# kostas1515/object_detectors

Measured on AMD Instinct MI355X. Metric: images/sec (fwd+bwd) YOLOv3 640px bs=32, higher is better.
Workload: dtype bf16; 1 GPU; YOLOv3 Darknet-53 training step (fwd+loss+bwd+SGD step), synthetic COCO 640px, per-GPU bs=32, 7 GT/img, random-init weights; global_batch=32, parallelism=dp1

## Files before the change

include/mi355det.h:

```cpp
#ifndef MI355DET_H
#define MI355DET_H

#include <stddef.h>
#include <stdint.h>

#ifdef __cplusplus
extern "C" {
#endif

#define MI355DET_OK 0
#define MI355DET_EINVAL (-1)
#define MI355DET_ELAUNCH (-2)
#define MI355DET_EWORKSPACE (-3)

#define MI355DET_MAX_SCALES 4
#define MI355DET_MAX_ANCHORS 8

const char* mi355det_last_error(void);
int mi355det_debug_set(int key, int value);
int mi355det_debug_ptr(int key, void* ptr);
int mi355det_version(void);

typedef struct {
  int32_t num_scales, na, num_classes, pad0;
// ... 156 lines not shown
                           void* workspace, size_t workspace_bytes, void* stream);

typedef struct {
  int32_t n, h, w, cin;
  int32_t ho, wo, cout;
  int32_t ksize, stride, pad;
  int32_t in_ld, out_ld;
} mi355det_conv_shape;

int mi355det_conv_fwd(const mi355det_conv_shape* s, const void* x, const void* w, const float* bias,
                      void* y, int out_f32, float* stats, int32_t cout_pad, void* stream);
typedef struct {
  const float* scale;
  const float* shift;
  const void* residual;
  int32_t residual_ld;
  int32_t relu;
  int64_t out_image_stride;
  float slope;
} mi355det_conv_epilogue;
int mi355det_conv_fwd_ex(const mi355det_conv_shape* s, const void* x, const void* w, const mi355det_conv_epilogue* e,
                         void* y, int out_f32, int32_t cout_pad, void* stream);
int mi355det_conv_autotune_mode(int on);

typedef struct {
  uint32_t table;
  int32_t value;
  uint64_t key;
} mi355det_tune_entry;
size_t mi355det_tune_export(void* buf, size_t cap);
int mi355det_tune_import(const void* buf, size_t bytes, int replace);
int mi355det_tune_lock(int on);
int mi355det_tune_clear(void);
int mi355det_conv_stats_rows(const mi355det_conv_shape* s, int32_t cout_pad);
int mi355det_stem_im2col(const float* img, void* out, int32_t n, int32_t h, int32_t w, void* stream);

int mi355det_stem_l1_rows(int32_t n, int32_t h, int32_t w);
int mi355det_stem_l1_fwd(const float* img, const void* w0, const float* scale_shift0, float slope, const void* w1, void* a0,
                         int32_t a0_ld, void* z1, int32_t z1_ld, float* stats, int32_t n, int32_t h, int32_t w, void* stream);
int mi355det_stem_l1_fwd_eval(const float* img, const void* w0, const float* scale_shift0, float slope, const void* w1,
                              const float* scale_shift1, void* a1, int32_t a1_ld, int32_t n, int32_t h, int32_t w, void* stream);
int mi355det_stem_rows(int32_t n, int32_t h, int32_t w);
int mi355det_stem_fwd_stats(const float* img, const void* w, float* partial, int32_t n, int32_t h, int32_t wd, void* stream);
int mi355det_stem_fwd_apply(const float* img, const void* w, const float* scale_shift, float slope, void* a, int32_t a_ld,
                            int32_t n, int32_t h, int32_t wd, void* stream);
int mi355det_stem_bwd_reduce(const float* img, const void* w, const float* scale_shift, float slope, const void* da,
// ... 385 lines not shown
```

include/mi355det_f16.h:

```cpp
#ifndef MI355DET_F16_H
#define MI355DET_F16_H
#include "mi355det.h"
#ifdef __cplusplus
extern "C" {
#endif

int mi355det_conv_autotune_mode_f16(int on);
int mi355det_conv_dgrad_f16(const mi355det_conv_shape* s, const void* dy, const void* wt, void* dx, const void* residual, int32_t residual_ld, void* stream);
int mi355det_conv_dgrad_bn_f16(const mi355det_conv_shape* s, const void* dy, const void* wt, void* dx, const void* residual, int32_t residual_ld, const void* z, int32_t z_ld, const float* scale_shift, float slope, float* partials, void* stream);
int mi355det_conv_dgrad_bn_rows_f16(const mi355det_conv_shape* s);
int mi355det_conv_dgrad_mask_f16(const mi355det_conv_shape* s, const void* dy, const void* wt, void* dx, const void* act, int32_t act_ld, const float* scale, int32_t relu, void* stream);
size_t mi355det_conv_dgrad_workspace_f16(const mi355det_conv_shape* s);
int mi355det_conv_dgrad_ws_f16(const mi355det_conv_shape* s, const void* dy, const void* wt, void* dx, const void* residual, int32_t residual_ld, void* workspace, size_t workspace_bytes, void* stream);
int mi355det_conv_fwd_f16(const mi355det_conv_shape* s, const void* x, const void* w, const float* bias, void* y, int out_f32, float* stats, int32_t cout_pad, void* stream);
int mi355det_conv_fwd_ex_f16(const mi355det_conv_shape* s, const void* x, const void* w, const mi355det_conv_epilogue* e, void* y, int out_f32, int32_t cout_pad, void* stream);
int mi355det_conv_stats_rows_f16(const mi355det_conv_shape* s, int32_t cout_pad);
int mi355det_debug_ptr_f16(int key, void* ptr);
int mi355det_debug_set_f16(int key, int value);
size_t mi355det_dgrad_pack_elems_f16(const mi355det_conv_shape* s);
int mi355det_pack_table_build_f16(const mi355det_pack_item* items, int32_t n, void* host_table, size_t host_bytes);
size_t mi355det_pack_table_bytes_f16(const mi355det_pack_item* items, int32_t n, int32_t* n_entries, int32_t* n_blocks);
int mi355det_pack_weights_f16(const mi355det_conv_shape* s, const float* w, int w_is_ohwi, void* w_fwd, int32_t cout_pad, void* w_dgrad, void* stream);
int mi355det_pack_weights_batched_f16(const void* dev_table, int32_t n_entries, int32_t n_blocks, void* stream);
int mi355det_stem_im2col_f16(const float* img, void* out, int32_t n, int32_t h, int32_t w, void* stream);
int mi355det_unpack_wgrad_f16(const mi355det_conv_shape* s, const float* dw, float* grad, void* stream);
int mi355det_conv_wgrad_f16(const mi355det_conv_shape* s, const void* x, const void* dy, float* dw, float* dbias, void* workspace, size_t workspace_bytes, void* stream);
int mi355det_conv_wgrad_autotune_f16(const mi355det_conv_shape* s, const void* x, const void* dy, float* dw, void* workspace, size_t workspace_bytes, void* stream);
size_t mi355det_conv_wgrad_workspace_f16(const mi355det_conv_shape* s);
int mi355det_add_bf16_f16(const void* a, int32_t a_ld, const void* b, int32_t b_ld, int32_t c, int64_t pixels, void* out, int32_t out_ld, void* stream);
int mi355det_bn_act_bwd_apply_f16(const void* g1, int32_t g1_ld, const void* g2, int32_t g2_ld, const void* z, int32_t z_ld, const float* scale_shift, const float* sums, const float* gamma, int32_t c, int64_t pixels, float slope, void* dz, int32_t dz_ld, float* dgamma, float* dbeta, void* stream);
// ... 24 lines not shown
```

object_detectors_amd/_lib.py:

```python
import ctypes as C
import os

HERE = os.path.dirname(os.path.abspath(__file__))
LIB_PATH = os.environ.get("MI355DET_LIB", os.path.join(HERE, "libmi355det.so"))

MAX_SCALES, MAX_ANCHORS = 4, 8

vp, i32, i64, f32, sz = C.c_void_p, C.c_int32, C.c_int64, C.c_float, C.c_size_t


class YoloGeom(C.Structure):
    _fields_ = [("num_scales", i32), ("na", i32), ("num_classes", i32), ("pad0", i32),
                ("img_size", f32), ("ignore_thr", f32), ("iou_type", i32), ("pad1", i32),
                ("grid", i32 * MAX_SCALES), ("off", i32 * (MAX_SCALES + 1)),
                ("anchor_w", (f32 * MAX_ANCHORS) * MAX_SCALES), ("anchor_h", (f32 * MAX_ANCHORS) * MAX_SCALES)]


class HeadView(C.Structure):
    _fields_ = [("ptr", vp), ("sb", i64), ("sc", i64), ("sp", i64)]


class YoloLossCfg(C.Structure):
    _fields_ = [("lambda_iou", f32), ("lambda_xy", f32), ("lambda_wh", f32), ("lambda_conf", f32),
                ("lambda_no_conf", f32), ("lambda_cls", f32), ("alpha", f32), ("gamma", f32),
# ... 99 lines not shown
    "mi355det_roi_align": (C.c_int, [vp, vp, vp, vp, i32, vp, i32, i32, i32, i32, i32, C.c_int, i32, i32, vp, vp, vp, vp]),
    "mi355det_topk": (C.c_int, [vp, i32, i64, i64, i32, f32, vp, vp, vp, vp]),
    "mi355det_conv_fwd": (C.c_int, [P(ConvShape), vp, vp, vp, vp, C.c_int, vp, i32, vp]),
    "mi355det_conv_dgrad": (C.c_int, [P(ConvShape), vp, vp, vp, vp, i32, vp]),
    "mi355det_conv_dgrad_mask": (C.c_int, [P(ConvShape), vp, vp, vp, vp, i32, vp, i32, vp]),
    "mi355det_conv_dgrad_workspace": (sz, [P(ConvShape)]),
    "mi355det_conv_dgrad_ws": (C.c_int, [P(ConvShape), vp, vp, vp, vp, i32, vp, sz, vp]),
    "mi355det_conv_wgrad_workspace": (sz, [P(ConvShape)]),
    "mi355det_conv_wgrad_autotune": (C.c_int, [P(ConvShape), vp, vp, vp, vp, sz, vp]),
    "mi355det_conv_wgrad": (C.c_int, [P(ConvShape), vp, vp, vp, vp, vp, sz, vp]),
    "mi355det_dgrad_pack_elems": (sz, [P(ConvShape)]),
    "mi355det_pack_weights": (C.c_int, [P(ConvShape), vp, C.c_int, vp, i32, vp, vp]),
    "mi355det_pack_table_bytes": (sz, [P(PackItem), i32, P(i32), P(i32)]),
    "mi355det_pack_table_build": (C.c_int, [P(PackItem), i32, vp, sz]),
    "mi355det_pack_weights_batched": (C.c_int, [vp, i32, i32, vp]),
    "mi355det_unpack_wgrad": (C.c_int, [P(ConvShape), vp, vp, vp]),
    "mi355det_gconv_pack_elems": (sz, [P(ConvShape), i32]),
    "mi355det_gconv_pack_weights": (C.c_int, [P(ConvShape), i32, vp, C.c_int, vp, vp, vp]),
    "mi355det_gconv_fwd_ex": (C.c_int, [P(ConvShape), i32, vp, vp, P(ConvEpilogue), vp, C.c_int, vp]),
    "mi355det_gconv_dgrad": (C.c_int, [P(ConvShape), i32, vp, vp, vp, vp]),
    "mi355det_gconv_wgrad_workspace": (sz, [P(ConvShape), i32]),
    "mi355det_gconv_wgrad": (C.c_int, [P(ConvShape), i32, vp, vp, vp, vp, sz, vp]),
    "mi355det_conv_autotune_mode": (C.c_int, [C.c_int]),
    "mi355det_tune_export": (sz, [vp, sz]),
    "mi355det_tune_import": (C.c_int, [vp, sz, C.c_int]),
    "mi355det_tune_lock": (C.c_int, [C.c_int]),
    "mi355det_tune_clear": (C.c_int, []),
    "mi355det_conv_stats_rows": (C.c_int, [P(ConvShape), i32]),
    "mi355det_stem_im2col": (C.c_int, [vp, vp, i32, i32, i32, vp]),
    "mi355det_stem_rows": (C.c_int, [i32, i32, i32]),
    "mi355det_stem_l1_rows": (C.c_int, [i32, i32, i32]),
    "mi355det_stem_l1_fwd": (C.c_int, [vp, vp, vp, f32, vp, vp, i32, vp, i32, vp, i32, i32, i32, vp]),
    "mi355det_stem_l1_fwd_eval": (C.c_int, [vp, vp, vp, f32, vp, vp, vp, i32, i32, i32, i32, vp]),
    "mi355det_stem_fwd_stats": (C.c_int, [vp, vp, vp, i32, i32, i32, vp]),
    "mi355det_stem_fwd_apply": (C.c_int, [vp, vp, vp, f32, vp, i32, i32, i32, i32, vp]),
    "mi355det_stem_bwd_reduce": (C.c_int, [vp, vp, vp, f32, vp, i32, vp, i32, i32, i32, vp]),
    "mi355det_stem_bwd_apply_wgrad": (C.c_int, [vp, vp, vp, vp, f32, vp, i32, vp, vp, vp, vp, i32, i32, i32, vp]),
    "mi355det_stem_bwd_fused": (C.c_int, [vp, vp, vp, f32, vp, i32, vp, vp, vp, i32, i32, i32, vp]),
    "mi355det_stem_bwd_finish": (C.c_int, [vp, vp, vp, vp, i64, vp, vp, vp, vp]),
    "mi355det_bn_finalize": (C.c_int, [vp, i32, i32, i32, i64, vp, vp, f32, f32, vp, vp, vp, vp]),
    "mi355det_bn_eval_scale_shift": (C.c_int, [i32, vp, vp, vp, vp, f32, vp, vp]),
    "mi355det_bn_fold_partials_f64": (C.c_int, [vp, i32, i32, i32, vp, vp]),
    "mi355det_bn_finalize_f64": (C.c_int, [vp, i32, i32, i64, vp, vp, f32, f32, vp, vp, vp, vp]),
    "mi355det_conv_dgrad_bn_rows": (C.c_int, [P(ConvShape)]),
    "mi355det_conv_dgrad_bn": (C.c_int, [P(ConvShape), vp, vp, vp, vp, i32, vp, i32, vp, C.c_float, vp, vp]),
    "mi355det_bn_bwd_sum_partials": (C.c_int, [vp, i32, i32, i32, vp, vp]),
# ... 174 lines not shown
```

object_detectors_amd/csrc/conv_kernels.hip:

```cpp
#include "common.h"

#include <cstdlib>

#include <unordered_map>

#include "tune_record.h"
#include "tune_timing.h"

using namespace mi355;

#include "igemm_common.h"

extern int g_wgrad_general;
extern int g_wgrad_force_dbg;
extern int g_wgrad8_off;
extern int g_wgrad_ablate;
extern int g_dgrad_s2_off;
extern int g_conv_strict;
int mi355det_internal_dgrad_s2(const mi355det_conv_shape* s, const void* dy, const void* wt, void* dx, const void* residual, int32_t residual_ld,
                               void* stream, int probe = 0);

namespace {

#define STAMP(v) do { if (PROF) { __builtin_amdgcn_sched_barrier(0); asm volatile("s_memtime %0\n\ts_waitcnt lgkmcnt(0)" : "=s"(v) :: "memory"); __builtin_amdgcn_sched_barrier(0); } } while (0)
// ... 80 lines not shown
      }
    }
    a_voff[i] = voff;
    a_valid[i] = vm;
  }
  if (PROF) asm volatile("s_nop 0" ::"v"(a_voff[0]), "v"(a_valid[A_PER - 1]));
  STAMP(t_p2);
  int b_voff[B_PER], b_instr[B_PER];
#pragma unroll
  for (int i = 0; i < B_PER; ++i) {
    const int instr = (wid * B_PER + i) % B_INSTR;
    const int row = instr * R + lrow;
    b_instr[i] = instr;
    b_voff[i] = (row * Ktot + (cpos ^ swz<BK>(row)) * 8) * 2;
  }
  __builtin_amdgcn_s_waitcnt(0xC07F);
  STAMP(t_p3);
  __builtin_amdgcn_s_barrier();
  STAMP(t_p4);

  const int cin_steps = __builtin_amdgcn_readfirstlane((p.ksplit > 1 ? p.Cin / p.ksplit : p.Cin) / BK);
  const int c0b = sp * cin_steps * (BK * 2);
  const int ksteps = ABL == 5 ? 0 : p.T * cin_steps;
  int pf_t = 0, pf_c = 0;

  auto stage = [&](int s, int buf) {
    const int coff = c0b + pf_c * (BK * 2);
    const int soff = __builtin_amdgcn_readfirstlane(s_toff[pf_t]) + coff;
    const int boff = pf_t * (p.Cin * 2) + coff;
    char* sa = smem + buf * STAGE;
    char* sb = sa + BM * ROWB;
#pragma unroll
    for (int i = 0; i < A_PER; ++i) {
      const int instr = wid * A_PER + i;
      bufld16(rsrc_x, sa + instr * 1024, ((a_valid[i] >> pf_t) & 1u) ? a_voff[i] : OOB_VOFF, soff);
    }
#pragma unroll
    for (int i = 0; i < B_PER; ++i) bufld16(rsrc_w, sb + b_instr[i] * 1024, b_voff[i], boff);
    if (++pf_c == cin_steps) {
      pf_c = 0;
      ++pf_t;
    }
  };

  auto issue_piece = [&](int q, int boff, int soff, int tap, int buf) {
    char* sa = smem + buf * STAGE;
    char* sb = sa + BM * ROWB;
    if (q < A_PER) {
      const int instr = wid * A_PER + q;
      bufld16(rsrc_x, sa + instr * 1024, ((a_valid[q] >> tap) & 1u) ? a_voff[q] : OOB_VOFF, soff);
    } else {
      bufld16(rsrc_w, sb + b_instr[q - A_PER] * 1024, b_voff[q - A_PER], boff);
    }
  };

  f32x4_t acc[TN][TM];
#pragma unroll
  for (int i = 0; i < TN; ++i)
#pragma unroll
    for (int j = 0; j < TM; ++j) acc[i][j] = {0.f, 0.f, 0.f, 0.f};

#pragma unroll
  for (int s = 0; s < D; ++s)
    if (s < ksteps && ABL != 1) stage(s, s);

  const int fr = lane & 15, fq = lane >> 4;
  int buf = 0;
  STAMP(t_loop);
  for (int s = 0; s < ksteps; ++s) {
    STAMP(t_a);
    const int younger = min(D - 1, ksteps - 1 - s);
    if (D >= 1 && younger >= D - 1) wait_vmcnt<(D - 1 > 0 ? D - 1 : 0) * PER>();
    else if (D >= 3 && younger == D - 2) wait_vmcnt<(D - 2 > 0 ? D - 2 : 0) * PER>();
    else if (D >= 4 && younger == D - 3) wait_vmcnt<(D - 3 > 0 ? D - 3 : 0) * PER>();
    else if (D >= 5 && younger == D - 4) wait_vmcnt<(D - 4 > 0 ? D - 4 : 0) * PER>();
    else if (D >= 6 && younger == D - 5) wait_vmcnt<(D - 5 > 0 ? D - 5 : 0) * PER>();
    else wait_vmcnt<0>();
    STAMP(t_b);
    __builtin_amdgcn_s_barrier();
    STAMP(t_c);
    const bool pf = s + D < ksteps;
    const int pbuf = buf == 0 ? NST - 1 : buf - 1;
    int il_soff = 0, il_tap = 0, il_boff = 0;
    if (!ILV) {
      if (pf && ABL != 1) stage(s + D, pbuf);
    } else if (pf) {
      il_tap = pf_t;
      il_soff = __builtin_amdgcn_readfirstlane(s_toff[pf_t]) + c0b + pf_c * (BK * 2);
      il_boff = pf_t * (p.Cin * 2) + c0b + pf_c * (BK * 2);
      if (++pf_c == cin_steps) {
        pf_c = 0;
        ++pf_t;
      }
    }
    STAMP(t_d);
    const char* sa = smem + buf * STAGE;
    const char* sb = sa + BM * ROWB;
#pragma unroll
    for (int ks = 0; ks < BK / 32; ++ks) {
      st16x8_t wf[TN], af[TM];
#pragma unroll
      for (int i = 0; i < TN; ++i) {
        const int row = wn * (TN * 16) + i * 16 + fr;
        if (ABL == 2) { wf[i] = __builtin_bit_cast(st16x8_t, make_uint4(row, s, ks, i)); asm volatile("" : "+v"(wf[i])); }
        else wf[i] = *(const st16x8_t*)(sb + row * ROWB + (((ks * 4 + fq) ^ swz<BK>(row)) << 4));
      }
#pragma unroll
      for (int j = 0; j < TM; ++j) {
        const int row = wm * (TM * 16) + j * 16 + fr;
        if (ABL == 2) { af[j] = __builtin_bit_cast(st16x8_t, make_uint4(row, s, ks, j)); asm volatile("" : "+v"(af[j])); }
        else af[j] = *(const st16x8_t*)(sa + row * ROWB + (((ks * 4 + fq) ^ swz<BK>(row)) << 4));
      }
      constexpr int NMF = TN * TM * (BK / 32);
      constexpr int G = NMF / PER > 0 ? NMF / PER : 1;
#pragma unroll
      for (int i = 0; i < TN; ++i)
// ... 303 lines not shown
      const int n = (int)fdiv((unsigned)t1, p.dMH), yy = t1 - n * p.MH;
      const int iy0 = yy * p.sin, ix0 = xx * p.sin;
      voff = ((((n - n_first) * p.Hin + iy0) * p.Win + ix0) * p.ldin + (cpos ^ swz<BK>(row)) * 8) * 2;
#pragma unroll
      for (int t = 0; t < MAX_TAPS; ++t) {
        const int dyt = (int)((p.dy_pack >> (4 * t)) & 0xF) - 2, dxt = (int)((p.dx_pack >> (4 * t)) & 0xF) - 2;
        const bool ok = t < p.T && (unsigned)(iy0 + dyt) < (unsigned)p.Hin && (unsigned)(ix0 + dxt) < (unsigned)p.Win;
        vm |= ok ? (1u << t) : 0u;
      }
    }
    a_voff[i] = voff;
    a_valid[i] = vm;
  }
#pragma unroll
  for (int i = 0; i < B_PER; ++i) {
    const int instr = (wid * B_PER + i) % B_INSTR;
    const int row = instr * R + lrow;
    b_instr[i] = instr;
    b_voff[i] = (row * Ktot + (cpos ^ swz<BK>(row)) * 8) * 2;
  }
  __builtin_amdgcn_s_waitcnt(0xC07F);
  __builtin_amdgcn_s_barrier();
  const int ksteps = Ktot / BK, cin_steps = p.Cin / BK;
  int pf_t = 0, pf_c = 0;

  f32x4_t acc[TN][TM];
#pragma unroll
  for (int i = 0; i < TN; ++i)
#pragma unroll
    for (int j = 0; j < TM; ++j) acc[i][j] = {0.f, 0.f, 0.f, 0.f};

  auto piece = [&](int q, int s, int soff, int tap, int buf, bool live) {
    char* sa = smem + buf * STAGE;
    char* sb = sa + BM * ROWB;
    if (q < A_PER) {
      const bool ok = live && ((a_valid[q] >> tap) & 1u);
      bufld16(rsrc_x, sa + (wid * A_PER + q) * 1024, ok ? a_voff[q] : OOB_VOFF, soff);
    } else {
      bufld16(rsrc_w, sb + b_instr[q - A_PER] * 1024, live ? b_voff[q - A_PER] : OOB_VOFF, s * (BK * 2));
    }
  };
  {
    const int soff = __builtin_amdgcn_readfirstlane(s_toff[0]);
#pragma unroll
    for (int q = 0; q < PER; ++q) piece(q, 0, soff, 0, 0, true);
    if (++pf_c == cin_steps) {
      pf_c = 0;
      ++pf_t;
    }
  }
  const int fr = lane & 15, fq = lane >> 4;
  for (int s = 0; s < ksteps; ++s) {
    const int buf = s & 1;
    wait_vmcnt<0>();
    __builtin_amdgcn_s_barrier();
    const bool live = s + 1 < ksteps;
    const int tap = live ? pf_t : 0;
    const int soff = __builtin_amdgcn_readfirstlane(s_toff[tap]) + pf_c * (BK * 2);
    if (++pf_c == cin_steps) {
      pf_c = 0;
      ++pf_t;
    }
    const char* sa = smem + buf * STAGE;
    const char* sb = sa + BM * ROWB;
    st16x8_t wf[KS][TN], af[KS][TM];
#pragma unroll
    for (int ks = 0; ks < KS; ++ks) {
#pragma unroll
      for (int i = 0; i < TN; ++i) {
        const int row = wn * (TN * 16) + i * 16 + fr;
        wf[ks][i] = *(const st16x8_t*)(sb + row * ROWB + (((ks * 4 + fq) ^ swz<BK>(row)) << 4));
      }
#pragma unroll
      for (int j = 0; j < TM; ++j) {
        const int row = wm * (TM * 16) + j * 16 + fr;
        af[ks][j] = *(const st16x8_t*)(sa + row * ROWB + (((ks * 4 + fq) ^ swz<BK>(row)) << 4));
      }
    }
#pragma unroll
    for (int ks = 0; ks < KS; ++ks)
#pragma unroll
      for (int i = 0; i < TN; ++i)
#pragma unroll
        for (int j = 0; j < TM; ++j) {
          acc[i][j] = MI355_MFMA_16x16x32(wf[ks][i], af[ks][j], acc[i][j]);
          const int cnt = (ks * TN + i) * TM + j + 1;
          if (cnt % G == 0 && cnt / G - 1 < PER) piece(cnt / G - 1, s + 1, soff, tap, buf ^ 1, live);
        }
    if (SCHED == 1) {
      __builtin_amdgcn_sched_group_barrier(0x100, KS * (TN + TM), 0);
#pragma unroll
      for (int q = 0; q < PER; ++q) {
        __builtin_amdgcn_sched_group_barrier(0x8, G, 0);
        __builtin_amdgcn_sched_group_barrier(0x20, 1, 0);
      }
    }
  }
  __builtin_amdgcn_s_waitcnt(0xC07F);
  wait_vmcnt<0>();
  __builtin_amdgcn_s_barrier();
  igemm_epilogue<WM, WN, TM, TN, EPI>(p, acc, smem, tid, NT, true, wm, wn, lane, mt, n0, m0);
}

__global__ void pack_fwd_kernel(const float* __restrict__ w, bf16_t* __restrict__ out, int cout, int cout_pad, int cin, int cin_pad, int kk,
                                long long s_co, long long s_ci, long long s_t) {
  const long long total = (long long)cout_pad * kk * cin_pad;
  for (long long i = blockIdx.x * (long long)blockDim.x + threadIdx.x; i < total; i += (long long)gridDim.x * blockDim.x) {
    const int c = (int)(i % cin_pad);
    const int t = (int)((i / cin_pad) % kk);
    const int co = (int)(i / ((long long)cin_pad * kk));
// ... 91 lines not shown
    const int co = (int)(j % cout), tap = (int)((j / cout) % T), r = (int)(j / ((long long)cout * T));
    const int px = r / cin, ci = r - px * cin;
    const int oy = py ? tap >> 1 : 0, ox = py ? tap & 1 : tap;
    const int kh = s2cat_k(py, oy), kw = s2cat_k(px, ox);
    float v = 0.f;
    if (kh >= 0 && kw >= 0) v = w[co * s_co + ci * s_ci + (kh * 3 + kw) * s_t];
    out[i] = f2s(v);
  }
}

bf16_t* g_zero_page = nullptr;

int ensure_zero_page() {
  if (g_zero_page) return 0;
  void* p = nullptr;
  if (hipMalloc(&p, 4096) != hipSuccess) return fail(MI355DET_ELAUNCH, "%s: hipMalloc(zero page) failed", "conv");
  if (hipMemset(p, 0, 4096) != hipSuccess) return fail(MI355DET_ELAUNCH, "%s: hipMemset(zero page) failed", "conv");
  g_zero_page = (bf16_t*)p;
  return 0;
}

unsigned long long* g_dbg = nullptr;

template <int WM, int WN, int TM, int TN, int BK, int NST, int EPI, bool PROF = false, bool ILV = false, int OCC = 0, int ABL = 0>
int launch_cfg(const IgemmParams& p_in, hipStream_t st) {
  IgemmParams p = p_in;
  p.dbg = PROF ? g_dbg : nullptr;
  constexpr int BM = WM * TM * 16, BN = WN * TN * 16;
  constexpr int lds_ring = NST * (BM + BN) * BK * 2 + 64;
  constexpr int lds_epi = EPI_LDS_OFF + WM * WN * (64 * (TN * 32 + 16) + 256);
  constexpr int lds = lds_ring > lds_epi ? lds_ring : lds_epi;
  const int gm = (p.M + BM - 1) / BM, gn = p.CoutPad / BN;
  auto k = igemm_kernel<WM, WN, TM, TN, BK, NST, EPI, PROF, ILV, OCC, ABL>;
  static DeviceOnce attr_done;
  attr_done.once([&] {
    (void)hipFuncSetAttribute((const void*)k, hipFuncAttributeMaxDynamicSharedMemorySize, lds);
  });
  hipLaunchKernelGGL(k, dim3(gm * gn * (p.ksplit > 1 ? p.ksplit : 1)), dim3(WM * WN * 64), lds, st, p);
  return check_launch("igemm");
}

template <int WM, int WN, int TM, int TN, int BK, int EPI, int SCHED>
int launch_il(const IgemmParams& p, hipStream_t st) {
  constexpr int BM = WM * TM * 16, BN = WN * TN * 16;
  constexpr int lds_ring = 2 * (BM + BN) * BK * 2 + 64;
  constexpr int lds_epi = EPI_LDS_OFF + WM * WN * (64 * (TN * 32 + 16) + 256);
  constexpr int lds = lds_ring > lds_epi ? lds_ring : lds_epi;
  const int gm = (p.M + BM - 1) / BM, gn = p.CoutPad / BN;
  auto k = igemm_il_kernel<WM, WN, TM, TN, BK, EPI, SCHED>;
  static DeviceOnce attr_done;
  attr_done.once([&] {
    (void)hipFuncSetAttribute((const void*)k, hipFuncAttributeMaxDynamicSharedMemorySize, lds);
  });
  hipLaunchKernelGGL(k, dim3(gm * gn), dim3(WM * WN * 64), lds, st, p);
  return check_launch("igemm_il");
}

int g_tune = 0;

int strict_reject(int cfg, const char* why) {
  char msg[160];
  snprintf(msg, sizeof(msg), "conv: forced tile configuration %d not taken: %s (strict mode, debug key 9)", cfg, why);
  return fail(MI355DET_EINVAL, "%s", msg);
}
bool strict_forced() { return g_conv_strict && g_tune != 0; }
TuneMap& g_igemm_tuned = tune_table(TUNE_IGEMM);
// ... 38 lines not shown
  auto k = igemm_dx_kernel<WM, WN, TM, TN, EPI, NSTB, PROF, BK>;
  static DeviceOnce attr_done;
  attr_done.once([&] {
    (void)hipFuncSetAttribute((const void*)k, hipFuncAttributeMaxDynamicSharedMemorySize, lds);
  });
  hipLaunchKernelGGL(k, dim3(gm * gn), dim3(WM * WN * 64), lds, st, p);
  return check_launch("igemm_dx");
}

enum CfgReq { REQ_WIDE, REQ_DX, REQ_IG8, REQ_NARROW, REQ_NARROW_DX };
typedef int (*LaunchFn)(const IgemmParams&, hipStream_t);
struct CfgRow {
  int id;
  unsigned epis;
  int req, a, b;
  bool tuned, solo;
  LaunchFn launch;
  bool narrow() const { return req == REQ_NARROW || req == REQ_NARROW_DX; }
};
constexpr unsigned eSTATS = 1u << EPI_STATS, eF32 = 1u << EPI_F32, eRES = 1u << EPI_RES, ePLAIN = 1u << EPI_PLAIN, eAFF = 1u << EPI_AFF,
                   eBNRED = 1u << EPI_BNRED, eALL = eSTATS | eF32 | eRES | ePLAIN | eAFF | eBNRED;

template <int EPI, int ROWS>
int launch_ig8(const IgemmParams& p, hipStream_t st) { return igemm8_launch(EPI, p, st, ROWS); }

template <int EPI>
int launch_narrow(const IgemmParams& p, hipStream_t st) {
  const bool k64 = p.Cin % 64 == 0;
  if (p.CoutPad % 64 == 0) return k64 ? launch_cfg<4, 1, 4, 4, 64, 2, EPI>(p, st) : launch_cfg<4, 1, 4, 4, 32, 3, EPI>(p, st);
  if (p.CoutPad % 32 == 0) return k64 ? launch_cfg<4, 1, 4, 2, 64, 2, EPI>(p, st) : launch_cfg<4, 1, 4, 2, 32, 4, EPI>(p, st);
  return fail(MI355DET_EINVAL, "%s: padded Cout must be a multiple of 32 (got %lld)", "conv", p.CoutPad);
}

#define CFG_ROW(id, epis, req, a, b, tuned, solo, ...) \
  {id, epis, req, a, b, tuned, solo, [] { if constexpr ((((epis) >> EPI) & 1u) != 0) return (LaunchFn)(__VA_ARGS__); else return (LaunchFn) nullptr; }()}

template <int EPI>
const CfgRow* cfg_rows() {
  static const CfgRow rows[] = {
    CFG_ROW( 0, eALL,                              REQ_NARROW,      0,   0, 1, 0, launch_narrow<EPI>),
    CFG_ROW( 1, eALL,                              REQ_WIDE,      128,   0, 1, 0, launch_cfg<2, 2, 4, 4, 64, 2, EPI>),
    CFG_ROW( 2, eALL,                              REQ_WIDE,      128,   0, 1, 0, launch_cfg<2, 2, 8, 4, 32, 2, EPI>),
    CFG_ROW( 3, eALL,                              REQ_WIDE,      256,   0, 1, 1, launch_cfg<2, 4, 8, 4, 64, 2, EPI>),
    CFG_ROW( 4, eALL,                              REQ_WIDE,      128,   0, 1, 0, launch_cfg<2, 2, 4, 4, 32, 3, EPI>),
    CFG_ROW( 5, eALL,                              REQ_WIDE,      128,   0, 1, 0, launch_cfg<2, 2, 4, 4, 32, 2, EPI, false, false, 4>),
    CFG_ROW( 6, eALL,                              REQ_WIDE,      256,   0, 1, 1, launch_il<2, 4, 8, 4, 64, EPI, 0>),
    CFG_ROW(15, eALL,                              REQ_DX,        128,  64, 1, 0, launch_dx<2, 2, 4, 4, EPI>),
// ... 177 lines not shown

}

extern "C" {

int mi355det_debug_set(int key, int value) {
  if (key == 0) g_tune = value;
  if (key == 1) g_wgrad_general = value;
  if (key == 2) g_dgrad_s2_off = value;
  if (key == 3) igemm8_set_dbg_mode(value);
  if (key == 8) g_wgrad8_off = value;
  if (key == 7) g_wgrad_force_dbg = value;
  if (key == 6) g_wgrad_ablate = value;
  if (key == 5) g_s2cat_force = value;
  if (key == 9) g_conv_strict = value;
  return 0;
}

int mi355det_conv_autotune_mode(int on) {
  g_autotune_mode = on != 0;
  return 0;
}

int mi355det_debug_ptr(int key, void* ptr) {
  if (key == 0) g_dbg = (unsigned long long*)ptr;
  if (key == 1) igemm8_set_dbg((unsigned long long*)ptr);
  return 0;
}

int mi355det_conv_stats_rows(const mi355det_conv_shape* s, int32_t cout_pad) {
  (void)cout_pad;
  return s ? (int)(((long long)s->n * s->ho * s->wo + 127) / 128) : 0;
}

static int conv_fwd_impl(const mi355det_conv_shape* s, const void* x, const void* w, const float* bias, void* y, int out_f32, float* stats,
                         int32_t cout_pad, const mi355det_conv_epilogue* ex, void* stream) {
  if (int e = check_shape(s, "conv_fwd")) return e;
  if (int e = ensure_zero_page()) return e;
  if (cout_pad < s->cout) return fail(MI355DET_EINVAL, "%s: cout_pad < cout", "conv_fwd");
  if (!out_f32 && (s->cout % 8)) return fail(MI355DET_EINVAL, "%s: 16-bit outputs need cout %% 8 == 0 (got %lld)", "conv_fwd", s->cout);
  IgemmParams p{};
  p.x = (const bf16_t*)x;
  p.w = (const bf16_t*)w;
  p.y = y;
  p.bias = bias;
  p.stats = stats;
// ... 521 lines not shown
```

object_detectors_amd/csrc/f16_names.h:

```cpp
#pragma once
#define mi355det_conv_autotune_mode mi355det_conv_autotune_mode_f16
#define mi355det_conv_dgrad mi355det_conv_dgrad_f16
#define mi355det_conv_dgrad_bn mi355det_conv_dgrad_bn_f16
#define mi355det_conv_dgrad_bn_rows mi355det_conv_dgrad_bn_rows_f16
#define mi355det_conv_dgrad_mask mi355det_conv_dgrad_mask_f16
#define mi355det_conv_dgrad_workspace mi355det_conv_dgrad_workspace_f16
#define mi355det_conv_dgrad_ws mi355det_conv_dgrad_ws_f16
#define mi355det_conv_fwd mi355det_conv_fwd_f16
#define mi355det_conv_fwd_ex mi355det_conv_fwd_ex_f16
#define mi355det_conv_stats_rows mi355det_conv_stats_rows_f16
#define mi355det_debug_ptr mi355det_debug_ptr_f16
#define mi355det_debug_set mi355det_debug_set_f16
#define mi355det_dgrad_pack_elems mi355det_dgrad_pack_elems_f16
#define mi355det_pack_table_build mi355det_pack_table_build_f16
#define mi355det_pack_table_bytes mi355det_pack_table_bytes_f16
#define mi355det_pack_weights mi355det_pack_weights_f16
#define mi355det_pack_weights_batched mi355det_pack_weights_batched_f16
#define mi355det_stem_im2col mi355det_stem_im2col_f16
#define mi355det_unpack_wgrad mi355det_unpack_wgrad_f16
#define mi355det_conv_wgrad mi355det_conv_wgrad_f16
#define mi355det_conv_wgrad_autotune mi355det_conv_wgrad_autotune_f16
#define mi355det_conv_wgrad_workspace mi355det_conv_wgrad_workspace_f16
#define mi355det_add_bf16 mi355det_add_bf16_f16
#define mi355det_bn_act_bwd_apply mi355det_bn_act_bwd_apply_f16
// ... 32 lines not shown
```

object_detectors_amd/csrc/igemm8_kernels.hip:

```cpp
#include "igemm_common.h"

struct SkParams {
  unsigned long long* dbg;
};

namespace {

typedef __attribute__((ext_vector_type(4))) unsigned u32x4_t;

constexpr int kBM = 256, kBN = 256, kBK = 64, kROWB = 128;
constexpr int kHALF = 128 * kROWB;
constexpr int kSTAGE = 4 * kHALF;
constexpr int kLDS = 2 * kSTAGE;

template <int N>
__device__ __forceinline__ void wait_vm() {
  asm volatile("s_waitcnt vmcnt(%0)" ::"n"(N) : "memory");
}
template <int PROF_>
__device__ __forceinline__ void bar_b() {
  if (PROF_ == 8) return;
  asm volatile("" ::: "memory");
  __builtin_amdgcn_s_barrier();
  asm volatile("" ::: "memory");
// ... 102 lines not shown
            for (int t = 0; t < MAX_TAPS; ++t) {
              if (t >= p.T) break;
              const int dyt = (int)((p.dy_pack >> (4 * t)) & 0xF) - 2, dxt = (int)((p.dx_pack >> (4 * t)) & 0xF) - 2;
              const bool ok = (unsigned)(iy0 + dyt) < (unsigned)p.Hin && (unsigned)(ix0 + dxt) < (unsigned)p.Win;
              vm |= ok ? (1u << t) : 0u;
            }
          }
          a_voff[h][i] = voff;
          a_valid[h][i] = vm;
        }
        {
          const int row = (r2 >> 5) * 64 + h * 32 + (r2 & 31);
          b_voff[h][i] = (row * Ktot + (cpos ^ sw) * 8) * 2;
        }
      }

    int xrd = (wm * 64 + fr) * kROWB + ((fq ^ fsw) << 4);
    int wrd = 2 * kHALF + (wn * 32 + fr) * kROWB + ((fq ^ fsw) << 4);

    auto tap_off = [&](int tap) {
      const int dyt = (int)((p.dy_pack >> (4 * tap)) & 0xF) - 2, dxt = (int)((p.dx_pack >> (4 * tap)) & 0xF) - 2;
      return ((dyt * p.Win + dxt) * p.ldin + p.tap_pad) * 2;
    };
    int pf_s = k0, pf_t = k0 / cin_steps, pf_c = k0 - pf_t * cin_steps;
    struct Slot { int tap, soffx, soffw, live; };
    auto next_slot = [&]() {
      Slot s;
      s.live = pf_s < k1;
      s.tap = s.live ? pf_t : 31;
      s.soffx = s.live ? tap_off(pf_t) + pf_c * (kBK * 2) : 0;
      s.soffw = s.live ? pf_s * (kBK * 2) : 0;
      ++pf_s;
      if (++pf_c == cin_steps) {
        pf_c = 0;
        ++pf_t;
      }
      return s;
    };
    auto issue_x = [&](const Slot& s, int h, int buf) {
      if (PROF == 3) return;
      char* dst = smem + buf * kSTAGE + h * kHALF + (2 * wid) * 1024;
#pragma unroll
      for (int i = 0; i < 2; ++i) bufld16(rsrc_x, dst + i * 1024, ((a_valid[h][i] >> s.tap) & 1u) ? a_voff[h][i] : OOB_VOFF, s.soffx);
    };
    auto issue_w = [&](const Slot& s, int h, int buf) {
      if (PROF == 3) return;
      char* dst = smem + buf * kSTAGE + (2 + h) * kHALF + (2 * wid) * 1024;
#pragma unroll
      for (int i = 0; i < 2; ++i) bufld16(rsrc_w, dst + i * 1024, s.live ? b_voff[h][i] : OOB_VOFF, s.soffw);
    };

    f32x4_t acc[TN][TM];
#pragma unroll
    for (int i = 0; i < TN; ++i)
#pragma unroll
      for (int j = 0; j < TM; ++j) acc[i][j] = {0.f, 0.f, 0.f, 0.f};

    Slot s1 = next_slot();
    issue_x(s1, 0, 0);
// ... 333 lines not shown
```

object_detectors_amd/csrc/igemm_common.h:

```cpp
#pragma once
#include "common.h"

using namespace mi355;

typedef __attribute__((ext_vector_type(4))) float f32x4_t;
typedef __attribute__((ext_vector_type(8))) unsigned short u16x8_t;

#define MAX_TAPS 9

struct FastDiv {
  unsigned mul, shift;
};
static FastDiv make_fastdiv(unsigned d) {
  FastDiv f;
  unsigned l = 0;
  while ((1ull << l) < d) ++l;
  f.shift = l;
  f.mul = (unsigned)(((1ull << 32) * ((1ull << l) - d)) / d + 1);
  return f;
}
__device__ __forceinline__ unsigned fdiv(unsigned n, const FastDiv f) { return (__umulhi(f.mul, n) + n) >> f.shift; }

struct IgemmParams {
  const bf16_t* x;
// ... 3 lines not shown
  const float* scale;
  int relu;
  long long ynstride;
  const bf16_t* z;
  const float* ss;
  int ldz;
  float slope;
  float* stats;
  const bf16_t* res;
  const bf16_t* zero;
  int M, MH, MW;
  int Hin, Win, ldin, Cin, sin;
  int Hout, Wout, ldout, so, oy0, ox0;
  int sox;
  int Cout, CoutPad, ldres;
  int T;
  int dy[MAX_TAPS], dx[MAX_TAPS];
  FastDiv dMW, dMH;
  int tap_pad;
  unsigned long long dy_pack, dx_pack;
  int ksplit;
  long long ysplit;
  int lin_in, lin_out;
  unsigned long long* dbg;
};

enum { EPI_STATS = 0, EPI_F32 = 1, EPI_RES = 2, EPI_PLAIN = 3, EPI_AFF = 4, EPI_BNRED = 5 };
#define EPI_LDS_OFF 4096
#define EPI_LDS_BYTES(nwaves) (EPI_LDS_OFF + (nwaves) * (64 * (8 * 16 * 2 + 16) + 256))

bool igemm8_applicable(const IgemmParams& p);
int igemm8_launch(int epi, const IgemmParams& p, hipStream_t st, int rows = 256);
void igemm8_set_dbg(unsigned long long* ptr);
void igemm8_set_dbg_mode(int mode);

namespace {

__device__ __forceinline__ void glds16(const void* gsrc, void* lds_dst_uniform) {
  __builtin_amdgcn_global_load_lds((const __attribute__((address_space(1))) void*)gsrc,
                                   (__attribute__((address_space(3))) void*)lds_dst_uniform, 16, 0, 0);
}

typedef __attribute__((ext_vector_type(4))) int srd_t;
__device__ __forceinline__ srd_t make_srd(const void* base, unsigned num_records) {
  const unsigned long long a = (unsigned long long)base;
  srd_t r;
// ... 329 lines not shown
```

Baseline: 1163 images/s.

## Add chunk-major K-loop ordering for implicit-GEMM convolutions

Introduces a KWalk abstraction so the K reduction in the implicit-GEMM conv kernels can iterate channel-chunk-major (all taps of a channel chunk, then the next chunk) instead of tap-major. This becomes the default whenever a conv has multiple taps and multiple channel chunks, except for stride-2 inputs with BK=32. The intent is better cache locality for activation loads, since consecutive K-steps then read neighbouring spatial positions of the same channel slice. The change adds extra index arithmetic per step, and the weight offset is now derived from tap and chunk rather than the linear step counter. The wgrad/dgrad kernels that take this path also depend on the packed weight layout matching the tap*Cin+chunk indexing.

```diff
diff --git a/include/mi355det.h b/include/mi355det.h
--- a/include/mi355det.h
+++ b/include/mi355det.h
@@ -202,6 +202,7 @@
 int mi355det_conv_fwd_ex(const mi355det_conv_shape* s, const void* x, const void* w, const mi355det_conv_epilogue* e,
                          void* y, int out_f32, int32_t cout_pad, void* stream);
 int mi355det_conv_autotune_mode(int on);
+int mi355det_conv_korder(int order);
 
 typedef struct {
   uint32_t table;
diff --git a/include/mi355det_f16.h b/include/mi355det_f16.h
--- a/include/mi355det_f16.h
+++ b/include/mi355det_f16.h
@@ -6,6 +6,7 @@
 #endif
 
 int mi355det_conv_autotune_mode_f16(int on);
+int mi355det_conv_korder_f16(int order);
 int mi355det_conv_dgrad_f16(const mi355det_conv_shape* s, const void* dy, const void* wt, void* dx, const void* residual, int32_t residual_ld, void* stream);
 int mi355det_conv_dgrad_bn_f16(const mi355det_conv_shape* s, const void* dy, const void* wt, void* dx, const void* residual, int32_t residual_ld, const void* z, int32_t z_ld, const float* scale_shift, float slope, float* partials, void* stream);
 int mi355det_conv_dgrad_bn_rows_f16(const mi355det_conv_shape* s);
diff --git a/object_detectors_amd/_lib.py b/object_detectors_amd/_lib.py
--- a/object_detectors_amd/_lib.py
+++ b/object_detectors_amd/_lib.py
@@ -145,6 +145,7 @@
     "mi355det_gconv_wgrad_workspace": (sz, [P(ConvShape), i32]),
     "mi355det_gconv_wgrad": (C.c_int, [P(ConvShape), i32, vp, vp, vp, vp, sz, vp]),
     "mi355det_conv_autotune_mode": (C.c_int, [C.c_int]),
+    "mi355det_conv_korder": (C.c_int, [C.c_int]),
     "mi355det_tune_export": (sz, [vp, sz]),
     "mi355det_tune_import": (C.c_int, [vp, sz, C.c_int]),
     "mi355det_tune_lock": (C.c_int, [C.c_int]),
diff --git a/object_detectors_amd/csrc/conv_kernels.hip b/object_detectors_amd/csrc/conv_kernels.hip
--- a/object_detectors_amd/csrc/conv_kernels.hip
+++ b/object_detectors_amd/csrc/conv_kernels.hip
@@ -126,25 +126,22 @@
   const int cin_steps = __builtin_amdgcn_readfirstlane((p.ksplit > 1 ? p.Cin / p.ksplit : p.Cin) / BK);
   const int c0b = sp * cin_steps * (BK * 2);
   const int ksteps = ABL == 5 ? 0 : p.T * cin_steps;
-  int pf_t = 0, pf_c = 0;
+  KWalk kw{0, 0};
 
   auto stage = [&](int s, int buf) {
-    const int coff = c0b + pf_c * (BK * 2);
-    const int soff = __builtin_amdgcn_readfirstlane(s_toff[pf_t]) + coff;
-    const int boff = pf_t * (p.Cin * 2) + coff;
+    const int tap = kw.tap;
+    const int soff = kslot_xoff(kw, __builtin_amdgcn_readfirstlane(s_toff[tap]), c0b, BK);
+    const int boff = kslot_woff(kw, p.Cin, c0b, BK);
     char* sa = smem + buf * STAGE;
     char* sb = sa + BM * ROWB;
 #pragma unroll
     for (int i = 0; i < A_PER; ++i) {
       const int instr = wid * A_PER + i;
-      bufld16(rsrc_x, sa + instr * 1024, ((a_valid[i] >> pf_t) & 1u) ? a_voff[i] : OOB_VOFF, soff);
+      bufld16(rsrc_x, sa + instr * 1024, ((a_valid[i] >> tap) & 1u) ? a_voff[i] : OOB_VOFF, soff);
     }
 #pragma unroll
     for (int i = 0; i < B_PER; ++i) bufld16(rsrc_w, sb + b_instr[i] * 1024, b_voff[i], boff);
-    if (++pf_c == cin_steps) {
-      pf_c = 0;
-      ++pf_t;
-    }
+    kwalk_next(kw, p.T, cin_steps, p.korder);
   };
 
   auto issue_piece = [&](int q, int boff, int soff, int tap, int buf) {
@@ -189,13 +186,10 @@
     if (!ILV) {
       if (pf && ABL != 1) stage(s + D, pbuf);
     } else if (pf) {
-      il_tap = pf_t;
-      il_soff = __builtin_amdgcn_readfirstlane(s_toff[pf_t]) + c0b + pf_c * (BK * 2);
-      il_boff = pf_t * (p.Cin * 2) + c0b + pf_c * (BK * 2);
-      if (++pf_c == cin_steps) {
-        pf_c = 0;
-        ++pf_t;
-      }
+      il_tap = kw.tap;
+      il_soff = kslot_xoff(kw, __builtin_amdgcn_readfirstlane(s_toff[kw.tap]), c0b, BK);
+      il_boff = kslot_woff(kw, p.Cin, c0b, BK);
+      kwalk_next(kw, p.T, cin_steps, p.korder);
     }
     STAMP(t_d);
     const char* sa = smem + buf * STAGE;
@@ -545,7 +539,7 @@
   __builtin_amdgcn_s_waitcnt(0xC07F);
   __builtin_amdgcn_s_barrier();
   const int ksteps = Ktot / BK, cin_steps = p.Cin / BK;
-  int pf_t = 0, pf_c = 0;
+  KWalk pf{0, 0};
 
   f32x4_t acc[TN][TM];
 #pragma unroll
@@ -553,24 +547,21 @@
 #pragma unroll
     for (int j = 0; j < TM; ++j) acc[i][j] = {0.f, 0.f, 0.f, 0.f};
 
-  auto piece = [&](int q, int s, int soff, int tap, int buf, bool live) {
+  auto piece = [&](int q, int woff, int soff, int tap, int buf, bool live) {
     char* sa = smem + buf * STAGE;
     char* sb = sa + BM * ROWB;
     if (q < A_PER) {
       const bool ok = live && ((a_valid[q] >> tap) & 1u);
       bufld16(rsrc_x, sa + (wid * A_PER + q) * 1024, ok ? a_voff[q] : OOB_VOFF, soff);
     } else {
-      bufld16(rsrc_w, sb + b_instr[q - A_PER] * 1024, live ? b_voff[q - A_PER] : OOB_VOFF, s * (BK * 2));
+      bufld16(rsrc_w, sb + b_instr[q - A_PER] * 1024, live ? b_voff[q - A_PER] : OOB_VOFF, woff);
     }
   };
   {
     const int soff = __builtin_amdgcn_readfirstlane(s_toff[0]);
 #pragma unroll
     for (int q = 0; q < PER; ++q) piece(q, 0, soff, 0, 0, true);
-    if (++pf_c == cin_steps) {
-      pf_c = 0;
-      ++pf_t;
-    }
+    kwalk_next(pf, p.T, cin_steps, p.korder);
   }
   const int fr = lane & 15, fq = lane >> 4;
   for (int s = 0; s < ksteps; ++s) {
@@ -578,12 +569,10 @@
     wait_vmcnt<0>();
     __builtin_amdgcn_s_barrier();
     const bool live = s + 1 < ksteps;
-    const int tap = live ? pf_t : 0;
-    const int soff = __builtin_amdgcn_readfirstlane(s_toff[tap]) + pf_c * (BK * 2);
-    if (++pf_c == cin_steps) {
-      pf_c = 0;
-      ++pf_t;
-    }
+    const int tap = live ? pf.tap : 0;
+    const int soff = live ? kslot_xoff(pf, __builtin_amdgcn_readfirstlane(s_toff[tap]), 0, BK) : 0;
+    const int woff = live ? kslot_woff(pf, p.Cin, 0, BK) : 0;
+    kwalk_next(pf, p.T, cin_steps, p.korder);
     const char* sa = smem + buf * STAGE;
     const char* sb = sa + BM * ROWB;
     st16x8_t wf[KS][TN], af[KS][TM];
@@ -608,7 +597,7 @@
         for (int j = 0; j < TM; ++j) {
           acc[i][j] = MI355_MFMA_16x16x32(wf[ks][i], af[ks][j], acc[i][j]);
           const int cnt = (ks * TN + i) * TM + j + 1;
-          if (cnt % G == 0 && cnt / G - 1 < PER) piece(cnt / G - 1, s + 1, soff, tap, buf ^ 1, live);
+          if (cnt % G == 0 && cnt / G - 1 < PER) piece(cnt / G - 1, woff, soff, tap, buf ^ 1, live);
         }
     if (SCHED == 1) {
       __builtin_amdgcn_sched_group_barrier(0x100, KS * (TN + TM), 0);
@@ -746,10 +735,18 @@
 
 unsigned long long* g_dbg = nullptr;
 
+int g_korder_force = -1;
+void set_korder(IgemmParams& p, int bk) {
+  const int cin_steps = (p.ksplit > 1 ? p.Cin / p.ksplit : p.Cin) / bk;
+  const bool split_lines_stride2 = bk == 32 && p.sin == 2;
+  p.korder = g_korder_force >= 0 ? g_korder_force : (split_lines_stride2 ? KORDER_TAP_MAJOR : korder_default(p.T, cin_steps));
+}
+
 template <int WM, int WN, int TM, int TN, int BK, int NST, int EPI, bool PROF = false, bool ILV = false, int OCC = 0, int ABL = 0>
 int launch_cfg(const IgemmParams& p_in, hipStream_t st) {
   IgemmParams p = p_in;
   p.dbg = PROF ? g_dbg : nullptr;
+  set_korder(p, BK);
   constexpr int BM = WM * TM * 16, BN = WN * TN * 16;
   constexpr int lds_ring = NST * (BM + BN) * BK * 2 + 64;
   constexpr int lds_epi = EPI_LDS_OFF + WM * WN * (64 * (TN * 32 + 16) + 256);
@@ -765,7 +762,9 @@
 }
 
 template <int WM, int WN, int TM, int TN, int BK, int EPI, int SCHED>
-int launch_il(const IgemmParams& p, hipStream_t st) {
+int launch_il(const IgemmParams& p_in, hipStream_t st) {
+  IgemmParams p = p_in;
+  set_korder(p, BK);
   constexpr int BM = WM * TM * 16, BN = WN * TN * 16;
   constexpr int lds_ring = 2 * (BM + BN) * BK * 2 + 64;
   constexpr int lds_epi = EPI_LDS_OFF + WM * WN * (64 * (TN * 32 + 16) + 256);
@@ -850,7 +849,11 @@
                    eBNRED = 1u << EPI_BNRED, eALL = eSTATS | eF32 | eRES | ePLAIN | eAFF | eBNRED;
 
 template <int EPI, int ROWS>
-int launch_ig8(const IgemmParams& p, hipStream_t st) { return igemm8_launch(EPI, p, st, ROWS); }
+int launch_ig8(const IgemmParams& p_in, hipStream_t st) {
+  IgemmParams p = p_in;
+  set_korder(p, 64);
+  return igemm8_launch(EPI, p, st, ROWS);
+}
 
 template <int EPI>
 int launch_narrow(const IgemmParams& p, hipStream_t st) {
@@ -1074,6 +1077,12 @@
   return 0;
 }
 
+int mi355det_conv_korder(int order) {
+  if (order < -1 || order > KORDER_CHUNK_MAJOR) return fail(MI355DET_EINVAL, "%s: order must be -1 (rule), 0 (tap-major) or 1 (chunk-major), got %lld", "conv_korder", order);
+  g_korder_force = order;
+  return 0;
+}
+
 int mi355det_debug_ptr(int key, void* ptr) {
   if (key == 0) g_dbg = (unsigned long long*)ptr;
   if (key == 1) igemm8_set_dbg((unsigned long long*)ptr);
diff --git a/object_detectors_amd/csrc/f16_names.h b/object_detectors_amd/csrc/f16_names.h
--- a/object_detectors_amd/csrc/f16_names.h
+++ b/object_detectors_amd/csrc/f16_names.h
@@ -1,5 +1,6 @@
 #pragma once
 #define mi355det_conv_autotune_mode mi355det_conv_autotune_mode_f16
+#define mi355det_conv_korder mi355det_conv_korder_f16
 #define mi355det_conv_dgrad mi355det_conv_dgrad_f16
 #define mi355det_conv_dgrad_bn mi355det_conv_dgrad_bn_f16
 #define mi355det_conv_dgrad_bn_rows mi355det_conv_dgrad_bn_rows_f16
diff --git a/object_detectors_amd/csrc/igemm8_kernels.hip b/object_detectors_amd/csrc/igemm8_kernels.hip
--- a/object_detectors_amd/csrc/igemm8_kernels.hip
+++ b/object_detectors_amd/csrc/igemm8_kernels.hip
@@ -148,19 +148,17 @@
       const int dyt = (int)((p.dy_pack >> (4 * tap)) & 0xF) - 2, dxt = (int)((p.dx_pack >> (4 * tap)) & 0xF) - 2;
       return ((dyt * p.Win + dxt) * p.ldin + p.tap_pad) * 2;
     };
-    int pf_s = k0, pf_t = k0 / cin_steps, pf_c = k0 - pf_t * cin_steps;
+    int pf_s = k0;
+    KWalk pf = kwalk_at(k0, p.T, cin_steps, p.korder);
     struct Slot { int tap, soffx, soffw, live; };
     auto next_slot = [&]() {
       Slot s;
       s.live = pf_s < k1;
-      s.tap = s.live ? pf_t : 31;
-      s.soffx = s.live ? tap_off(pf_t) + pf_c * (kBK * 2) : 0;
-      s.soffw = s.live ? pf_s * (kBK * 2) : 0;
+      s.tap = s.live ? pf.tap : 31;
+      s.soffx = s.live ? kslot_xoff(pf, tap_off(pf.tap), 0, kBK) : 0;
+      s.soffw = s.live ? kslot_woff(pf, p.Cin, 0, kBK) : 0;
       ++pf_s;
-      if (++pf_c == cin_steps) {
-        pf_c = 0;
-        ++pf_t;
-      }
+      kwalk_next(pf, p.T, cin_steps, p.korder);
       return s;
     };
     auto issue_x = [&](const Slot& s, int h, int buf) {
diff --git a/object_detectors_amd/csrc/igemm_common.h b/object_detectors_amd/csrc/igemm_common.h
--- a/object_detectors_amd/csrc/igemm_common.h
+++ b/object_detectors_amd/csrc/igemm_common.h
@@ -1,5 +1,6 @@
 #pragma once
 #include "common.h"
+#include "korder.h"
 
 using namespace mi355;
 
@@ -49,6 +50,7 @@
   int ksplit;
   long long ysplit;
   int lin_in, lin_out;
+  int korder;
   unsigned long long* dbg;
 };
 
diff --git a/object_detectors_amd/csrc/korder.h b/object_detectors_amd/csrc/korder.h
--- /dev/null
+++ b/object_detectors_amd/csrc/korder.h
@@ -0,0 +1,44 @@
+#pragma once
+
+#if defined(__HIPCC__) || defined(__CUDACC__)
+#define KORDER_HD __host__ __device__ __forceinline__
+#else
+#define KORDER_HD inline
+#endif
+
+enum { KORDER_TAP_MAJOR = 0, KORDER_CHUNK_MAJOR = 1 };
+
+struct KWalk {
+  int tap, chunk;
+};
+
+KORDER_HD KWalk kwalk_at(int s, int T, int cin_steps, int order) {
+  KWalk k;
+  if (order == KORDER_CHUNK_MAJOR) {
+    k.chunk = s / T;
+    k.tap = s - k.chunk * T;
+  } else {
+    k.tap = s / cin_steps;
+    k.chunk = s - k.tap * cin_steps;
+  }
+  return k;
+}
+
+KORDER_HD void kwalk_next(KWalk& k, int T, int cin_steps, int order) {
+  if (order == KORDER_CHUNK_MAJOR) {
+    if (++k.tap == T) {
+      k.tap = 0;
+      ++k.chunk;
+    }
+  } else {
+    if (++k.chunk == cin_steps) {
+      k.chunk = 0;
+      ++k.tap;
+    }
+  }
+}
+
+KORDER_HD int kslot_xoff(const KWalk& k, int tap_off, int c0b, int bk) { return tap_off + c0b + k.chunk * (bk * 2); }
+KORDER_HD int kslot_woff(const KWalk& k, int cin, int c0b, int bk) { return (k.tap * cin + k.chunk * bk) * 2 + c0b; }
+
+KORDER_HD int korder_default(int T, int cin_steps) { return (T > 1 && cin_steps > 1) ? KORDER_CHUNK_MAJOR : KORDER_TAP_MAJOR; }
```

Result: no change. 1169 images/s, median of 6 (+0.5%).
